# pfeiferd/genestrip

Measured on AMD Instinct MI355X. Metric: Gbp/s classified (match goal), k=31, 150bp reads; bit-exact CSV counts, higher is better.
Workload: dtype int64; 1 GPU; match: 10000000 synthetic 150 bp reads per GPU, k=31, 1911550-k-mer / 20-taxid store resident in HBM (BASELINE.json configs[1]); reads_per_gpu=10000000, read_len=150, k=31, store_kmers=1911550, store_record_bytes=67108864, store_table_bytes=131072, gate_bytes=524288, parallelism=read-sharded x1, store replicated

## Files before the change

### genestrip_amd/__init__.py

```python
from .binding import (
    GsError, lib, lib_path, device_count, abi_version, DeviceKMerStore, MatchConfig, FastqKMerMatcher,
    DeviceBloomFilter, BloomInfo, requested_mask, FastqBloomFilter, DeviceDbBuilder, DeviceDbQuality, DeviceDbUpdater, DeviceDbSizer, plan_ranges, kmer_ranges, N_COLS, N_DCOLS, N_SUMS, COLS, MEM_HOST, MEM_DEVICE,
    F_FOUND, F_RETURNED, F_COUNTED, BLOOM_XOR, BLOOM_MURMUR, BLOOM_BLOCKED, ABI_SYMBOLS, calibrate, bgzf_members, inflate_members, gunzip_device, deflate_device, deflate_reference, BGZF_EOF, DeviceDeflater, deflate_bound, DeviceReads, KrakenCounter, DeviceGenomes, DeviceView, DeviceAccessionMap, accession_slots, slot_accessions, DeviceTaxTree, read_taxids, RANK_NAMES,
    CAL_VALU_PURE, CAL_VALU_MIX, CAL_SALU, CAL_VALU_SALU, CAL_VMEM_BYTES, CAL_VMEM_WORDS, CAL_VMEM_SHARED_LINES,
    CAL_VMEM_SCATTERED, CAL_RANDOM_LINES,
)

__all__ = [
    "GsError", "lib", "lib_path", "device_count", "abi_version", "DeviceKMerStore", "MatchConfig",
    "FastqKMerMatcher", "DeviceReads", "KrakenCounter", "DeviceAccessionMap", "accession_slots", "slot_accessions", "DeviceTaxTree", "read_taxids", "RANK_NAMES", "DeviceBloomFilter", "BloomInfo", "requested_mask", "FastqBloomFilter", "DeviceDbBuilder", "DeviceDbQuality", "DeviceDbUpdater",
    "DeviceDbSizer", "DeviceGenomes", "plan_ranges", "kmer_ranges",
]
```

### genestrip_amd/binding.py

```python
import ctypes as C
import os
import sys

import numpy as np

_HERE = os.path.dirname(os.path.abspath(__file__))
_LIB = None

N_COLS, N_DCOLS, N_SUMS = 10, 4, 7
COLS = ("reads", "kmers from reads", "kmers", "unique kmers", "contigs", "contig len sq sum", "max contig length",
        "reads >=1 kmer", "reads bps", "max contig read no")
MEM_HOST, MEM_DEVICE = 0, 1
F_FOUND, F_RETURNED, F_COUNTED = 1, 2, 4
BLOOM_XOR, BLOOM_MURMUR, BLOOM_BLOCKED = 0, 1, 2

ABI_SYMBOLS = (
    "gs_last_error", "gs_strerror", "gs_device_cache_trim", "gs_abi_version", "gs_device_count",
    "gs_match_merge", "gs_match_max_contig_reads", "gs_db_create", "gs_db_get_info", "gs_db_destroy", "gs_db_save", "gs_db_load",
    "gs_match_begin", "gs_match_submit", "gs_match_submit_async", "gs_match_wait", "gs_match_sync", "gs_match_finish", "gs_match_reset", "gs_match_destroy",
    "gs_match_device_state", "gs_match_or_bitmap", "gs_match_kernel_time", "gs_match_prefilter_info", "gs_match_sn_info", "gs_match_segments",
    "gs_match_segments_fetch", "gs_match_max_counts", "gs_db_create_striped", "gs_db_create_stripe", "gs_db_stripe_export", "gs_db_stripe_attach", "gs_db_load_striped", "gs_db_load_stripe", "gs_dbbuild_begin", "gs_dbbuild_set_range", "gs_dbbuild_add", "gs_dbbuild_finish", "gs_dbbuild_fetch", "gs_dbbuild_to_db", "gs_dbbuild_destroy", "gs_db_create_part", "gs_match_encode", "gs_match_probe_keys", "gs_match_encode_route", "gs_match_route_geometry", "gs_unroute_region", "gs_match_reduce", "gs_route_keys",
    "gs_unroute_nodes",
    "gs_match_submit_text", "gs_match_submit_fasta", "gs_match_submit_fastq_ml", "gs_match_text_wait_copy", "gs_match_text_status", "gs_match_text_clear_error",
    "gs_match_text_select", "gs_match_segments_text", "gs_match_text_newlines", "gs_match_text_read_bounds", "gs_match_text_line_classes",
    "gs_pinned_alloc", "gs_pinned_free",
    "gs_filter_submit_text", "gs_filter_text_wait_copy", "gs_filter_text_status", "gs_filter_text_reset",
    "gs_filter_submit_fasta", "gs_filter_submit_fastq_ml", "gs_filter_text_read_bounds", "gs_filter_text_line_classes",
    "gs_bloom_create", "gs_bloom_build", "gs_bloom_get", "gs_bloom_destroy",
    "gs_bloom_build_db", "gs_bloom_get_info", "gs_bloom_save", "gs_bloom_load", "gs_filter_submit", "gs_filter_sync", "gs_filter_kernel_time",
    "gs_calibrate",
    "gs_match_get_device", "gs_inflate_members", "gs_inflater_create", "gs_inflater_feed", "gs_inflater_tail", "gs_gunzipper_open", "gs_gunzipper_reopen", "gs_gunzipper_next", "gs_gunzipper_info", "gs_gunzipper_first_span", "gs_gunzipper_park", "gs_gunzipper_close", "gs_gunzip_plan_device", "gs_gunzip_free", "gs_gunzip_device", "gs_text_cut_device", "gs_device_fetch", "gs_inflater_fetch", "gs_filter_get_device", "gs_inflater_reset", "gs_inflater_destroy", "gs_inflate_last_error",
    "gs_filter_compact_text", "gs_match_compact_text", "gs_filter_compact_records", "gs_match_compact_records", "gs_match_kraken_records", "gs_match_set_taxids", "gs_match_kraken_text", "gs_match_kraken_time", "gs_deflater_create", "gs_deflater_pack", "gs_deflater_info", "gs_deflater_destroy", "gs_deflater_append", "gs_deflater_pending", "gs_deflater_flush",
    "gs_deflate_bound", "gs_deflate_host", "gs_deflate_host_reference", "gs_deflate_last_error", "gs_match_text_descriptors", "gs_match_submit_fixed",
    "gs_db_value_counts", "gs_dbexport_create", "gs_dbexport_fetch", "gs_dbexport_get_device", "gs_dbexport_fastq_begin",
    "gs_dbexport_fastq_next", "gs_dbexport_destroy",
# ... 69 lines not shown
        raise GsError(-6, f"{path} is missing: build it with `make -C genestrip_amd/csrc` (hipcc, gfx950); "
                          "genestrip_amd has no CPU fallback")
    _preload_hip_runtime()
    L = C.CDLL(path)
    vp, i32, i64, dbl, ci = C.c_void_p, C.c_int32, C.c_int64, C.c_double, C.c_int
    sig = {
        "gs_last_error": (C.c_char_p, []), "gs_strerror": (C.c_char_p, [ci]), "gs_device_cache_trim": (ci, []), "gs_abi_version": (ci, []),
        "gs_device_count": (ci, [vp]),
        "gs_db_create": (ci, [vp, ci, ci, i64, vp, vp, i32, vp]), "gs_db_get_info": (ci, [vp, vp]),
        "gs_db_destroy": (ci, [vp]), "gs_db_save": (ci, [vp, C.c_char_p]), "gs_db_load": (ci, [vp, ci, C.c_char_p]),
        "gs_match_begin": (ci, [vp, vp, vp]), "gs_match_submit": (ci, [vp, vp, vp, i64, i64, ci, vp, vp]),
        "gs_match_submit_async": (ci, [vp, vp, vp, i64, i64, vp, vp, vp]), "gs_match_wait": (ci, [vp, i64]),
        "gs_match_sync": (ci, [vp]), "gs_match_finish": (ci, [vp, vp, vp]), "gs_match_reset": (ci, [vp]),
        "gs_match_destroy": (ci, [vp]), "gs_match_device_state": (ci, [vp, vp, vp, vp, vp, vp]),
        "gs_match_or_bitmap": (ci, [vp, vp, i64]), "gs_match_merge": (ci, [vp, ci]), "gs_match_max_contig_reads": (ci, [vp, vp]), "gs_match_kernel_time": (ci, [vp, vp, vp]), "gs_match_prefilter_info": (ci, [vp, vp]), "gs_match_sn_info": (ci, [vp, vp]),
        "gs_db_create_part": (ci, [vp, ci, ci, i64, vp, vp, i32, vp, ci, ci]),
        "gs_db_create_striped": (ci, [vp, vp, ci, ci, i64, vp, vp, i32, vp]),
        "gs_db_create_stripe": (ci, [vp, ci, ci, ci, ci, i64, vp, vp, i32, vp]),
        "gs_db_stripe_export": (ci, [vp, vp]),
        "gs_db_stripe_attach": (ci, [vp, ci, vp]),
        "gs_db_load_striped": (ci, [vp, vp, ci, C.c_char_p]),
        "gs_db_load_stripe": (ci, [vp, ci, ci, ci, C.c_char_p]),
        "gs_dbbuild_begin": (ci, [vp, ci, ci, i32, vp, ci, ci, ci]),
        "gs_dbbuild_add": (ci, [vp, vp, vp, vp, i64, ci, ci]),
        "gs_dbbuild_set_range": (ci, [vp, C.c_uint64, C.c_uint64]),
        "gs_dbbuild_finish": (ci, [vp, vp]),
        "gs_dbbuild_fetch": (ci, [vp, vp, vp]),
        "gs_dbbuild_to_db": (ci, [vp, vp]),
        "gs_dbbuild_destroy": (ci, [vp]),
        "gs_dbquality_begin": (ci, [vp, vp, ci, ci, ci]),
# ... 141 lines not shown
def _check(rc):
    if rc != 0:
        raise GsError(rc, (lib().gs_last_error() or b"").decode(errors="replace"))


def abi_version():
    return lib().gs_abi_version()


def device_count():
    n = C.c_int(0)
    rc = lib().gs_device_count(C.byref(n))
    return n.value if rc == 0 else 0


class InflateMember(C.Structure):
    _fields_ = [("payload_offset", C.c_int64), ("payload_len", C.c_uint32), ("isize", C.c_uint32), ("crc32", C.c_uint32),
                ("reserved", C.c_uint32)]


def bgzf_members(data):
    import struct
    b = bytes(data) if not isinstance(data, (bytes, bytearray)) else data
    out, o, n = [], 0, len(b)
    while o + 28 <= n and b[o] == 0x1f and b[o + 1] == 0x8b and b[o + 2] == 8 and (b[o + 3] & 4):
        if b[o + 3] & ~4:
            break
        xlen = struct.unpack_from("<H", b, o + 10)[0]
        q, bsize = o + 12, None
        while q + 4 <= o + 12 + xlen:
# ... 940 lines not shown
    def kernel_time(self):
        n, ms = C.c_int64(0), C.c_double(0)
        _check(lib().gs_match_kernel_time(self.h, C.byref(n), C.byref(ms)))
        return n.value, ms.value

    def prefilter_info(self):
        info = (C.c_int64 * 4)()
        _check(lib().gs_match_prefilter_info(self.h, info))
        return {"built": bool(info[0]), "n_lmers": int(info[1]), "survivors": int(info[2]), "reads": int(info[3])}

    def sn_info(self):
        info = (C.c_int64 * 3)()
        _check(lib().gs_match_sn_info(self.h, info))
        return {"deferred": bool(info[0]), "booked": int(info[1]), "rows": int(info[2])}

    def close(self):
        if getattr(self, "h", None):
            lib().gs_match_destroy(self.h)
            self.h = None

    def __del__(self):
        try:
            self.close()
        except Exception:
            pass


class BloomInfo(C.Structure):
    _fields_ = [("kind", C.c_int32), ("k", C.c_int32), ("n_hashes", C.c_int32), ("pad", C.c_int32), ("bits", C.c_int64),
                ("n_words", C.c_int64), ("expected_insertions", C.c_int64), ("n_inserted", C.c_int64), ("fpp", C.c_double)]
# ... 622 lines not shown
```

### genestrip_amd/csrc/gs_api.cpp

```cpp
#include <hip/hip_runtime.h>
#include <sys/mman.h>
#include <unistd.h>

#include <algorithm>
#include <atomic>
#include <chrono>
#include <cmath>
#include <cstdio>
#include <cstdlib>
#include <cstring>
#include <memory>
#include <string>
#include <thread>
#include <utility>
#include <vector>

#include "gs_absmod.h"
#include "gs_checksum.h"
#include "gs_indexfile.h"
#include "gs_launch.h"
#include "gs_layout.h"
#include "gs_params.h"
#include "gs_prefilter.h"
#include "gs_taxparse.h"
// ... 2052 lines not shown
    u64 *d_stat_rec_count = nullptr;
    size_t stat_recs_cap = 0;
    int32_t *d_stat_vi = nullptr;
    size_t stat_vi_cap = 0;
    bool use_stat_recs = false;
    GsQuotTable *d_quot = nullptr, *h_quot = nullptr;
    hipEvent_t quot_copied = nullptr;
    int pf_mode = -1;
    uint32_t *pf_h = nullptr;
    int64_t pf_slot_reads[4] = {0, 0, 0, 0};
    bool pf_slot_pending[4] = {false, false, false, false};
    int64_t pf_batches = 0;
    int pf_pause = 0;
    int64_t pf_last_survivors = -1, pf_last_reads = 0;
    int pf_last_slot = -1;
    int sn_mode = -1;
    bool sn_lds = false;
    GsSnRec *d_sn_recs = nullptr;
    size_t sn_recs_cap = 0;
    uint16_t *d_sn_nodes = nullptr;
    size_t sn_nodes_cap = 0;
    uint32_t *d_sn_list = nullptr;
    size_t sn_list_cap = 0;
    bool sn_last = false;
    int quot_max = 0;
    double quot_tax = 0, quot_class = 0;
    int stat_copies = 1;
    bool stats_spread = false;
    uint32_t *d_hit_counts = nullptr;
    uint32_t *d_bitmap = nullptr;
// ... 524 lines not shown
        for (int b = 0; b < 2; b++) {
            stage_free(g.bank[b]);
            if (g.copied[b]) hipEventDestroy(g.copied[b]);
        }
        for (hipEvent_t ev : g.finished)
            if (ev) hipEventDestroy(ev);
    }
    if (run->stream) hipStreamDestroy(run->stream);
    delete run;
}

#define GS_PF_MAX_PASS 0.5
#define GS_PF_HIT_RICH 0.85
#define GS_PF_PAUSE 15
#define GS_PF_SLOTS 4
static bool prefilter_rule(const gs_db *db, int mode, int samples) {
    if (mode == 0 || !db->d_pf || db->pf_set < 0) return false;
    if (mode > 0) return true;
    return 1.0 - std::pow(1.0 - (double)db->pf_set / (double)(1LL << 29), (double)samples) < GS_PF_MAX_PASS;
}
static bool prefilter_eligible(const gs_db *db) { return db->d_rec != nullptr && !db->striped() && db->n_parts <= 1 && db->info.k >= GS_MIN_K; }

static int db_ensure_prefilter(gs_db *db, int mode) {
    if (mode == 0 || db->pf_set >= 0 || !prefilter_eligible(db)) return GS_OK;
    const size_t l1_words = (size_t)1 << (GS_PF_L1_BITS - 5);
    hipStream_t stream = nullptr;
    HIP_TRY(hipStreamCreateWithFlags(&stream, hipStreamNonBlocking));
    u64 *d_count = nullptr;
    u64 count = 0;
    hipError_t e = gs_dev_alloc((void **)&db->d_pf, sizeof(uint32_t) * (GS_PF_L2_WORDS + l1_words));
    if (e == hipSuccess) e = gs_dev_alloc((void **)&d_count, sizeof(u64));
    if (e == hipSuccess) e = hipMemsetAsync(db->d_pf, 0, sizeof(uint32_t) * (GS_PF_L2_WORDS + l1_words), stream);
    if (e == hipSuccess) e = hipMemsetAsync(d_count, 0, sizeof(u64), stream);
    if (e == hipSuccess) {
// ... 33 lines not shown
    if (cfg->max_paths < 1 || cfg->max_paths > 128) return fail(GS_E_INVALID, "max_paths must be in [1,128] (C/GSConfigKey.java:350)");
    HIP_TRY(hipSetDevice(db->device));
    if (!db->complete()) return fail(GS_E_STATE, "striped store: not every stripe is attached yet (gs_db_stripe_attach)");
    if (cfg->count_unique && db->unique_owner && !db->striped())
        return fail(GS_E_STATE, "this store already has an active unique-counting run (the seen bits live in the table)");
    int pf_mode = -1;
    if (const char *ev = getenv("GS_PREFILTER")) pf_mode = atoi(ev) != 0 ? 1 : 0;
    {
        const int prc = db_ensure_prefilter(db, pf_mode);
        if (prc) return prc;
    }
    gs_run *run = new gs_run();
    run->db = db;
    run->cfg = *cfg;
    run->pf_mode = pf_mode;
    if (const char *ev = getenv("GS_SN_DEFER")) run->sn_mode = atoi(ev) != 0 ? 1 : 0;
    const size_t nv = (size_t)db->info.n_values;
    run->bitmap_words = (db->n_slots() + 31) / 32 + db->n_rec;
    hipError_t e = hipStreamCreateWithFlags(&run->stream, hipStreamNonBlocking);
    const char *force_global = getenv("GS_FORCE_GLOBAL_STATS");
    if (nv > GS_NV_LDS || (force_global != nullptr && atoi(force_global) != 0)) {
        int copies = 16;
        if (const char *ev = getenv("GS_STAT_COPIES")) copies = std::max(1, std::min(64, atoi(ev)));
        while (copies > 1 && (size_t)copies * nv * 96 > ((size_t)64 << 20)) copies /= 2;
        run->stat_copies = copies;
        run->use_stat_recs = nv <= GS_STAT_REC_MAX_VALUES;
        if (const char *ev = getenv("GS_STAT_RECS")) run->use_stat_recs = run->use_stat_recs && atoi(ev) != 0;
    }
    else {
        run->stat_copies = 16;
// ... 192 lines not shown
        if (run->db->info.n_values > 640 && (rc = grow(&run->d_stat_vi, &run->stat_vi_cap, (size_t)rec_room, run->stream))) return rc;
        if (!run->d_stat_rec_count) HIP_TRY(gs_dev_alloc((void **)&run->d_stat_rec_count, sizeof(u64)));
        HIP_TRY(hipMemsetAsync(run->d_stat_rec_count, 0, sizeof(u64), run->stream));
        P.stat_recs = run->d_stat_recs;
        P.stat_rec_count = (unsigned long long *)run->d_stat_rec_count;
    }
    const bool huge = !d_nodes && (off_stride != 0 || fixed_len - run->db->info.k + 1 >= run->huge_min);
    const bool no_queues = off_stride == 0 && !d_nodes && fixed_len - run->db->info.k + 1 <= 128 && !huge;
    if (!no_queues) HIP_TRY(hipMemsetAsync(run->d_long_count, 0, 6 * sizeof(unsigned int), run->stream));
    if (huge && (rc = ensure_huge(run, &P))) return rc;
    run->pf_last_survivors = -1;
    run->pf_last_reads = n_reads;
    run->pf_last_slot = -1;
    bool prefilter = P.quot != nullptr && fixed_len - run->db->info.k + 1 >= 65 && !d_skip && no_queues &&
                     prefilter_rule(run->db, run->pf_mode, gs_pf_samples(fixed_len, run->db->info.k));
    if (prefilter && run->pf_mode < 0) {
        for (int i = 0; i < GS_PF_SLOTS; i++)
            if (run->pf_slot_pending[i] && run->pf_h[i] != 0xffffffffu) {
                run->pf_slot_pending[i] = false;
                if ((double)run->pf_h[i] > GS_PF_HIT_RICH * (double)run->pf_slot_reads[i]) run->pf_pause = GS_PF_PAUSE;
            }
        if (run->pf_pause > 0) {
            run->pf_pause--;
            prefilter = false;
        }
    }
    run->sn_last = false;
    if (P.quot != nullptr && run->sn_lds && run->sn_mode != 0 && run->cfg.max_paths <= 64 && P.db.n_parts <= 1 && !d_skip &&
        P.db.n_values <= GS_SN_CODE_MAX && grow(&run->d_sn_recs, &run->sn_recs_cap, (size_t)n_reads, run->stream) == GS_OK &&
        grow(&run->d_sn_list, &run->sn_list_cap, (size_t)n_reads, run->stream) == GS_OK &&
        grow(&run->d_sn_nodes, &run->sn_nodes_cap, (size_t)n_reads * GS_SN_ROW, run->stream) == GS_OK) {
        P.sn_recs = run->d_sn_recs;
        P.sn_nodes = run->d_sn_nodes;
        run->sn_last = true;
    }
    int pf_slot = -1;
    if (prefilter) {
        if (!run->pf_h) {
            HIP_TRY(hipHostMalloc((void **)&run->pf_h, sizeof(uint32_t) * GS_PF_SLOTS, hipHostMallocDefault));
            for (int i = 0; i < GS_PF_SLOTS; i++) run->pf_h[i] = 0;
        }
    }
    if (prefilter || P.sn_recs)
        HIP_TRY(hipMemsetAsync(run->d_long_count + (prefilter ? 6 : 7), 0, sizeof(unsigned int) * ((prefilter ? 1 : 0) + (P.sn_recs ? 2 : 0)), run->stream));
    if ((rc = timer_start(run->timer, run->cfg.profile != 0, run->stream))) return rc;
    if (prefilter) {
        GsPrefilterParams F{};
        F.seq = d_seq;
        F.n_reads = n_reads;
// ... 2637 lines not shown
    return GS_OK;
}

extern "C" int gs_match_sn_info(gs_run *run, int64_t *info) {
    if (!run || !info) return fail(GS_E_INVALID, "NULL argument");
    HIP_TRY(hipSetDevice(run->db->device));
    HIP_TRY(hipStreamSynchronize(run->stream));
    info[0] = run->sn_last ? 1 : 0;
    info[1] = info[2] = 0;
    if (run->sn_last) {
        uint32_t n[2] = {0, 0};
        HIP_TRY(hipMemcpy(n, run->d_long_count + 7, sizeof(n), hipMemcpyDeviceToHost));
        info[1] = (int64_t)n[0];
        info[2] = (int64_t)n[1];
    }
    return GS_OK;
}

extern "C" int gs_match_kernel_time(gs_run *run, int64_t *launches, double *total_ms) {
    if (!run) return fail(GS_E_INVALID, "run is NULL");
    HIP_TRY(hipSetDevice(run->db->device));
    HIP_TRY(hipStreamSynchronize(run->stream));
    int rc = timer_collect(run->timer);
    if (rc) return rc;
    if (launches) *launches = run->timer.launches;
    if (total_ms) *total_ms = run->timer.total_ms;
    return GS_OK;
}

struct gs_bloom {
// ... 2424 lines not shown
```

### genestrip_amd/csrc/gs_kernels.hip

```cpp
#include <hip/hip_runtime.h>
#include <stdint.h>

#include <algorithm>
#include <type_traits>

#include "gs_launch.h"
#include "gs_layout.h"
#include "gs_params.h"
#include "gs_wave.h"

#define GS_LONG_CHUNK 64
#define GS_LONG_NONE 0xffffffffu

#if GS_PHASE
extern "C" int gs_debug_phase(unsigned long long *out, int reset) {
    if (out && hipMemcpyFromSymbol(out, HIP_SYMBOL(gs_phase_acc), sizeof(unsigned long long) * 16) != hipSuccess) return -1;
    if (reset) {
        unsigned long long z[16] = {0};
        if (hipMemcpyToSymbol(HIP_SYMBOL(gs_phase_acc), z, sizeof(z)) != hipSuccess) return -1;
    }
    return 0;
}
#endif

// ... 23 lines not shown

__device__ __forceinline__ bool gs_anc_or_self(int a_tin, int a_tout, int x_tin) { return a_tin <= x_tin && x_tin < a_tout; }

template <typename Tree>
__device__ __forceinline__ int gs_lca(const Tree &t, int a, int b) {
    if (a == b) return a;
    if (a < 0 || b < 0) return -1;
    const int tb = t.tin[b];
    while (a >= 0 && !gs_anc_or_self(t.tin[a], t.tout[a], tb)) a = t.parent[a];
    return a;
}

__device__ __forceinline__ int gs_sc_load(const int32_t *p) { return __hip_atomic_load(p, __ATOMIC_RELAXED, __HIP_MEMORY_SCOPE_AGENT); }
__device__ __forceinline__ void gs_sc_store(int32_t *p, int v) { __hip_atomic_store(p, v, __ATOMIC_RELAXED, __HIP_MEMORY_SCOPE_AGENT); }

template <bool LONG, bool FROM_NODES, int KC, bool WIDE, bool REC, bool STRIPED, int CTX = 2, bool FIXED = false>
__device__ __forceinline__ void gs_process_read(const GsMatchParams &P, const GsStats &st, int64_t r, u64 off, int L,
                                                int lane, int (*s_dvi)[128], int (*s_dcnt)[128], int wave_in_block,
                                                int32_t *tag, int32_t *cnt, int serial, const uint32_t (&pre)[3],
                                                uint32_t *wave_g, unsigned long long *cur, u64 live1 = 0, int64_t slot = 0) {
    static_assert(!FIXED || (!LONG && !FROM_NODES), "one iteration, probed here");
    const GsDbDev &db = P.db;
    const int k = KC ? KC : db.k;
    const int max = L - k + 1;
    const uint8_t *rd = P.seq + off;
    int out_class = -1;
    int out_flags = 0;

    if (FIXED || max > 0) {
        const int64_t read_no = P.first_read_no + r;
        const u64 key_lo = ((1ULL << 40) - 1) - ((u64)read_no & ((1ULL << 40) - 1));
        const int n_iter = LONG ? (max + 127) >> 7 : 1;
        bool found = false;
        int n_miss = 0, bad_lo = 0;
        bool bad_hi = false;
        int carry_last = GS_NODE_NONE;
// ... 46 lines not shown
                const u64 pb = P.pos_off[r] + (u64)base;
#pragma unroll
                for (int s = 0; s < 2; s++) {
                    const int p = base + 64 * s + lane;
                    int v = p < max ? P.nodes[pb + 64 * s + lane] : GS_NODE_NONE;
                    if (p < max && (v >= db.n_values || v < GS_NODE_INVALID)) v = GS_NODE_MISS;
                    node[s] = v;
                }
            } else {
                const GsMark mk = {P.count_unique, P.hit_counts, STRIPED ? P.bitmap : nullptr,
                                   STRIPED ? P.bitmap + ((db.bucket_mask + 1) * GS_SLOTS_PER_BUCKET >> 5) : nullptr};
#ifndef GS_AGG_ALL
#define GS_AGG_ALL 0
#endif
                const u64 live[2] = {~0ULL, live1};
                gs_probe_planes<KC, STRIPED, CTX, (REC || GS_AGG_ALL) && !LONG, 2, FIXED>(db, Bhi, Blo, Bbad, base, max, lane, node, wave_g, mk, FIXED ? live : nullptr);
            }

            if (!LONG) GS_STAMP(5, node[0] ^ node[1])
            const u64 hit0 = __ballot(node[0] >= 0), hit1 = __ballot(node[1] >= 0);
            found = found || ((hit0 | hit1) != 0);
            n_miss += __popcll(__ballot(node[0] == GS_NODE_MISS)) + __popcll(__ballot(node[1] == GS_NODE_MISS));

            u64 m0 = hit0, m1 = hit1;
#define GS_FIRST_NODE()                                                                                   \
    {                                                                                                     \
        const int j = m0 ? __builtin_ctzll(m0) : 64 + __builtin_ctzll(m1);                                \
        one_vi = j < 64 ? gs_readlane(node[0], j) : gs_readlane(node[1], j - 64);                         \
        const u64 e0 = __ballot(node[0] == one_vi), e1 = __ballot(node[1] == one_vi);                     \
        one_cnt = __popcll(e0) + __popcll(e1);                                                            \
        m0 &= ~e0;                                                                                        \
// ... 535 lines not shown
        s_cur[wave_in_block][0] = 0;
        s_cur[wave_in_block][1] = 64;
    }
    GS_STRIPE_TABLE((const GsMatchParams *)kp0)
#if GS_PHASE
    if (lane < 16) gs_phase_row()[lane] = 0;
    __builtin_amdgcn_fence(__ATOMIC_RELEASE, "wavefront");
    __builtin_amdgcn_wave_barrier();
    gs_stamp(-1);
#endif
    constexpr bool CAN_FIX = !FROM_NODES && !WIDE && !STRIPED;
    const int fixed_L = P.fixed_len;
    const bool fixed_batch = CAN_FIX && P.off_stride == 0 && fixed_L >= 128 && fixed_L - k + 1 <= 128 && P.quot != nullptr &&
                             (!LDS_STATS || (P.sn_recs != nullptr && P.sn_nodes != nullptr));
    const u64 fixed_live1 = gs_low_mask(fixed_L - k + 1 - 64);
    auto reads = [&](auto fixed) {
        constexpr bool FIXED = decltype(fixed)::value;
        const int64_t po_step = n_waves * P.off_stride;
        const uint64_t *po = P.off + wave_id * P.off_stride;
        uint32_t trips = 0;
        typedef const __attribute__((address_space(4))) uint32_t *GsSurvPtr;
        int64_t n_trips = n_reads;
        if (P.surv_list != nullptr) n_trips = (int64_t)*(GsSurvPtr)P.surv_count;
        if (FIXED && wave_id < n_trips) trips = (uint32_t)(n_trips - wave_id - 1) / (uint32_t)n_waves + 1u;
        const GsSurvPtr sl0 = FIXED ? (GsSurvPtr)P.surv_list : nullptr;
        for (int64_t t = wave_id; FIXED ? trips != 0 : t < n_trips; t += n_waves, po += po_step, trips--) {
            GsKernargPtr kp = kp0;
#ifndef GS_KERNARG_HOISTED
            asm volatile("" : "+s"(kp));
#endif
            const GsMatchParams &Q = *(const GsMatchParams *)kp;
            int64_t r = t;
// ... 12 lines not shown
                L = (int)(po[1] - off);
            }
            GS_STAMP(0, L)
            if (!FIXED && L - k + 1 > 128) continue;
            uint32_t pre[3];
            const uint8_t *rd = Q.seq + off;
            if (FIXED) {
                pre[0] = rd[lane];
                pre[1] = rd[64 + lane];
                const uint32_t c2 = rd[128 + lane < L ? 128 + lane : L - 1];
                pre[2] = 128 + lane < L ? c2 : GS_FILL;
            } else {
#pragma unroll
                for (int w = 0; w < 3; w++) pre[w] = 64 * w + lane < L ? rd[64 * w + lane] : GS_FILL;
            }
            gs_process_read<false, FROM_NODES, KC, WIDE, !LDS_STATS, STRIPED, CTX, FIXED>(Q, st, r, off, L, lane, s_dvi, s_dcnt, wave_in_block, nullptr, nullptr, 0,
                                                                                          pre, s_g[wave_in_block], s_cur[wave_in_block], fixed_live1, t);
        }
    };
    if constexpr (CAN_FIX) {
        if (fixed_batch)
            reads(std::true_type());
        else
            reads(std::false_type());
    } else
        reads(std::false_type());
#if GS_PHASE
    __builtin_amdgcn_fence(__ATOMIC_ACQUIRE, "wavefront");
    if (lane < 15) atomicAdd(&gs_phase_acc[lane], gs_phase_row()[lane]);
#endif
    if (!LDS_STATS && P.stat_recs != nullptr) {
        __builtin_amdgcn_fence(__ATOMIC_ACQUIRE, "wavefront");
        const u64 base = s_cur[wave_in_block][0], used = s_cur[wave_in_block][1];
        if (used < 64 && (u64)lane >= used) P.stat_recs[base + (u64)lane].vi = -1;
    }
    GS_STATS_EPILOGUE()
}

template <int NS, int KC, int CTX>
__device__ __forceinline__ void gs_process_read_wide(const GsMatchParams &P, const GsStats &st, int64_t r, u64 off, int L, int lane, uint32_t *wave_g) {
    int *s_dvi = reinterpret_cast<int *>(wave_g), *s_dcnt = reinterpret_cast<int *>(wave_g) + 64 * NS;
// ... 882 lines not shown
}

template <bool FROM_NODES, int KC, bool WIDE, bool STRIPED, int CTX>
static void gs_launch_match_t(const GsMatchParams *P, int grid, size_t lds, bool lds_stats, hipStream_t stream) {
    if (lds_stats)
        hipLaunchKernelGGL((gs_match_kernel<true, FROM_NODES, KC, WIDE, STRIPED, CTX>), dim3(grid), dim3(GS_BLOCK), lds, stream, *P);
    else
        hipLaunchKernelGGL((gs_match_kernel<false, FROM_NODES, KC, WIDE, STRIPED, CTX>), dim3(grid), dim3(GS_BLOCK), lds, stream, *P);
}

extern "C" hipError_t gs_launch_match(const GsMatchParams *P, int grid, hipStream_t stream) {
    const size_t lds = gs_stats_lds_bytes(P->db.n_values);
    const bool lds_stats = P->db.n_values <= GS_NV_LDS && !gs_force_global_stats();
    const bool ctx = P->db.mgate_ctx != 0;
    if (P->sn_nodes != nullptr && (!lds_stats || P->db.n_values > GS_SN_CODE_MAX)) return hipErrorInvalidValue;
    if (P->db.n_parts > 1) {
        if (P->nodes != nullptr) return hipErrorInvalidValue;
        if (P->max_paths > 64)
            gs_launch_match_t<false, 0, true, true, 2>(P, grid, lds, lds_stats, stream);
        else if (P->db.k == 31)
            ctx ? gs_launch_match_t<false, 31, false, true, 1>(P, grid, lds, lds_stats, stream)
                : gs_launch_match_t<false, 31, false, true, 0>(P, grid, lds, lds_stats, stream);
        else
            ctx ? gs_launch_match_t<false, 0, false, true, 1>(P, grid, lds, lds_stats, stream)
                : gs_launch_match_t<false, 0, false, true, 0>(P, grid, lds, lds_stats, stream);
        return hipGetLastError();
    }
    if (P->nodes != nullptr) {
        if (P->max_paths > 64)
            gs_launch_match_t<true, 0, true, false, 0>(P, grid, lds, lds_stats, stream);
// ... 185 lines not shown
```

### genestrip_amd/csrc/gs_params.h

```cpp
#pragma once
#include <stdint.h>

#include "../../include/gsgpu.h"
#include "gs_layout.h"
#include "gs_snrec.h"

#define GS_BLOCK 256
#ifndef GS_NV_LDS
#define GS_NV_LDS 128
#endif
#define GS_NV_TREE_LDS 2048
#define GS_STAT_REC_MAX_VALUES 10240

struct GsStatRec {
    int32_t vi;
    int32_t contigs;
    int64_t kmers;
    int64_t sq;
    uint64_t max_key;
    int32_t counted;
    int32_t read_kmers;
    int32_t read_len;
    int32_t n_pos;
    int32_t tax_err;
// ... 11 lines not shown
    int32_t classify, count_unique, max_paths, threshold;
    double max_read_tax_err, max_read_class_err;
    int64_t *sums;
    int64_t *max_keys;
    double *dsums;
    uint32_t *bitmap;
    uint32_t *hit_counts;
    int32_t *class_vi;
    uint8_t *flags;
    unsigned int *long_count;
    uint32_t *long_list;
    const int32_t *nodes;
    const unsigned long long *pos_off;
    int32_t off_stride;
    int32_t fixed_len;
    int32_t pad0;
    int32_t stat_copies;
    const uint32_t *skip;
    const GsQuotTable *quot;
    GsStatRec *stat_recs;
    unsigned long long *stat_rec_count;
    unsigned int *huge_count;
    uint32_t *huge_list;
    struct GsHugeHead *huge_head;
    struct GsHugeChunk *huge_chunks;
    uint32_t *huge_cnt;
    uint32_t *huge_first;
    uint32_t *huge_touch;
    uint32_t *huge_fold;
    int64_t long_cap;
    int32_t wide_mask;
// ... 381 lines not shown
```

### genestrip_amd/csrc/gs_wave.h

```cpp
#pragma once
#include <hip/hip_runtime.h>
#include <stdint.h>

#include "gs_layout.h"
#include "gs_params.h"

#ifndef GS_ABLATE
#define GS_ABLATE 0
#endif

#define GS_NODE_MISS (-1)
#define GS_NODE_INVALID (-2)
#define GS_NODE_NONE (-3)

__device__ __forceinline__ int gs_lane() { return (int)__lane_id(); }
__device__ __forceinline__ int gs_readlane(int v, int l) { return __builtin_amdgcn_readlane(v, l); }
__device__ __forceinline__ int gs_rfl(int v) { return __builtin_amdgcn_readfirstlane(v); }
__device__ __forceinline__ unsigned long long gs_bitset0(unsigned long long x, int bit) {
    asm("s_bitset0_b64 %0, %1" : "+s"(x) : "s"(bit));
    return x;
}
template <int LANE>
__device__ __forceinline__ int gs_writelane(int old, int v) {
    asm("v_writelane_b32 %0, %1, %2" : "+v"(old) : "s"(v), "n"(LANE));
// ... 241 lines not shown
#pragma unroll
        for (int d = 0; d < ND; d++) g[d] = (KC || d < w) ? row[d] : 0xffffffffu;
        __builtin_amdgcn_sched_group_barrier(0x100, (ND + 1) / 2, 0);
        uint32_t mn = g[0];
#pragma unroll
        for (int d = 1; d < ND; d++) mn = g[d] < mn ? g[d] : mn;
        __builtin_amdgcn_sched_group_barrier(0x002, ND, 0);
        const int idx = (int)(mn & 0xffu) + ((TWO && s >= 2) ? 128 : 0);
        cf[s] = wave_g[CAN + idx];
        p[s] = idx - (64 * s + lane);
    }
    __builtin_amdgcn_wave_barrier();
}

__device__ __forceinline__ u64 gs_low_mask(int n) { return n >= 64 ? ~0ULL : (n <= 0 ? 0ULL : ((1ULL << n) - 1ULL)); }
template <int KC, bool STRIPED, int CTX = 2, bool AGG = false, int NS = 2, bool LIT = false>
__device__ __forceinline__ void gs_probe_planes(const GsDbDev &db, const u64 (&Bhi)[NS + 1], const u64 (&Blo)[NS + 1],
                                                const u64 (&Bbad)[NS + 1], int base, int max, int lane, int (&node)[NS],
                                                uint32_t *wave_g, const GsMark &mk, const u64 *live = nullptr) {
    static_assert(NS == 2 || !AGG, "the seen-bit accumulators are laid out for two sub-rounds");
    const int k = KC ? KC : db.k;
    const uint32_t kmask = (1u << k) - 1u;
    const uint32_t vmask2 = 2u * ((1u << db.vbits) - 1u);
    const int shift_rem = (int)db.vbits + 3;
    const uint32_t bmask = (uint32_t)db.bucket_mask;
    bool any_bad = false;
#pragma unroll
    for (int w = 0; w <= NS; w++) any_bad = any_bad || Bbad[w] != 0;
    uint32_t fhi[NS], flo[NS];
    u64 act[NS];
#pragma unroll
    for (int s = 0; s < NS; s++) {
        const u64 vm = live != nullptr ? live[s] : gs_low_mask(max - base - 64 * s);
        fhi[s] = (uint32_t)gs_funnel(Bhi[s], Bhi[s + 1], lane) & kmask;
        flo[s] = (uint32_t)gs_funnel(Blo[s], Blo[s + 1], lane) & kmask;
        act[s] = vm;
        node[s] = GS_ACT(vm) ? GS_NODE_MISS : GS_NODE_NONE;
        if (any_bad) {
            const u64 wb = __ballot(((uint32_t)gs_funnel(Bbad[s], Bbad[s + 1], lane) & kmask) != 0u) & vm;
            act[s] = vm & ~wb;
            node[s] = GS_ACT(wb) ? GS_NODE_INVALID : node[s];
        }
    }
    if (db.mgate != nullptr) {
        int mp[NS];
        uint32_t cf[NS];
        GS_STAMP(2, fhi[1] ^ flo[1])
        uint32_t rhi[NS], rlo[NS];
#pragma unroll
        for (int s = 0; s < NS; s++) {
            rhi[s] = __brev(fhi[s]) >> (32 - k);
            rlo[s] = (__brev(flo[s]) >> (32 - k)) ^ kmask;
        }
        gs_wave_minimizers<KC, NS, LIT>(Bhi, Blo, fhi, flo, rhi, rlo, k, lane, wave_g, mp, cf);
        GS_STAMP(3, cf[0] ^ cf[1])
        uint32_t gh[NS], ohi[NS], olo[NS];
        int j[NS];
#pragma unroll
        for (int s = 0; s < NS; s++) gs_min_oriented_cf(cf[s], fhi[s], flo[s], rhi[s], rlo[s], k, mp[s], gh[s], ohi[s], olo[s], j[s]);
        const bool use_hint = STRIPED || CTX == 1 || (CTX == 2 && db.mgate_ctx);
        u64 two[NS];
#pragma unroll
        for (int s = 0; s < NS; s++) two[s] = ~0ULL;
        if ((GS_ABLATE & 4) == 0) {
            uint32_t gw[NS];
            uint32_t gk[NS];
#pragma unroll
            for (int s = 0; s < NS; s++) gk[s] = (CTX == 1 || (CTX == 2 && db.mgate_ctx)) ? gs_gate_ctx_key(gh[s], ohi[s], olo[s], j[s], k) : gh[s];
#pragma unroll
            for (int s = 0; s < NS; s++)
                gw[s] = db.mgate[GS_ACT(act[s]) ? ((CTX == 1 || (CTX == 2 && db.mgate_ctx)) ? gs_mgate_word_ctx(gk[s], db.mgate_bits) : gs_mgate_word(gk[s], db.mgate_bits)) : 0u];
#pragma unroll
            for (int s = 0; s < NS; s++) {
                const uint32_t bits = gs_mgate_bits(gk[s]);
                act[s] &= __ballot((gw[s] & bits) == bits);
                if (use_hint) two[s] = __ballot((gw[s] & gs_mgate_hint(gk[s])) != 0u);
            }
            GS_STAMP(4, gw[0] ^ gw[1])
        }
        if (GS_ABLATE & 6) {
#pragma unroll
            for (int s = 0; s < NS; s++)
                if (GS_ACT(act[s]) && (gh[s] ^ ohi[s] ^ olo[s] ^ (uint32_t)j[s]) == 0x12345u) node[s] = 0;
            return;
        }
        if (STRIPED || db.rec != nullptr) {
            u64 any_act = 0;
#pragma unroll
            for (int s = 0; s < NS; s++) any_act |= act[s];
            if (any_act == 0) return;
            if (AGG && mk.count_unique) {
#pragma unroll
                for (int q = 0; q < 5; q++) wave_g[64 * q + lane] = 0u;
                __builtin_amdgcn_fence(__ATOMIC_RELEASE, "wavefront");
                __builtin_amdgcn_wave_barrier();
            }
#pragma unroll
            for (int s = 0; s < NS; s++) {
                bool pending = false;
                if (GS_ACT(act[s])) {
                    const uint32_t jj = (uint32_t)j[s];
// ... 102 lines not shown
```

### include/gsgpu.h

```cpp
#ifndef GSGPU_H
#define GSGPU_H

#include <stdint.h>
#include <stddef.h>

#ifdef __cplusplus
extern "C" {
#endif

#define GS_ABI_VERSION 3

enum {
    GS_OK = 0,
    GS_E_INVALID = -1,
    GS_E_NOMEM = -2,
    GS_E_HIP = -3,
    GS_E_UNSUPPORTED = -4,
    GS_E_STATE = -5,
    GS_E_NODEVICE = -6,
    GS_E_IO = -7,
    GS_E_CANCELLED = -8
};

enum { GS_MEM_HOST = 0, GS_MEM_DEVICE = 1, GS_MEM_DEVICE_TEXT = 2  };
// ... 228 lines not shown
int gs_unroute_nodes(gs_run *run, const uint64_t *keys, const uint32_t *idx, const int32_t *back, int64_t n_routed,
                     int32_t *nodes, int64_t n_keys);

int gs_match_segments(gs_run *run, const uint8_t *seq, const uint64_t *offsets, int64_t n_reads, int mem,
                      uint64_t *seg_off);
int gs_match_segments_fetch(gs_run *run, int32_t *codes, int32_t *starts);
int gs_match_segments_text(gs_run *run, uint64_t *seg_off);
int gs_match_text_newlines(gs_run *run, uint32_t *newlines);
int gs_match_text_descriptors(gs_run *run, const int64_t *records, int32_t n, uint8_t *out, int32_t stride);
int gs_match_text_read_bounds(gs_run *run, uint64_t *bounds);

int gs_match_kernel_time(gs_run *run, int64_t *launches, double *total_ms);

int gs_match_prefilter_info(gs_run *run, int64_t *info);
int gs_match_sn_info(gs_run *run, int64_t *info);
int gs_match_get_device(gs_run *run, int *device);

typedef struct gs_bloom gs_bloom;
enum { GS_BLOOM_XOR = 0, GS_BLOOM_MURMUR = 1, GS_BLOOM_BLOCKED = 2 };

int gs_bloom_create(gs_bloom **out, int device, int kind, int64_t bits, int32_t n_hashes,
                    const int64_t *hash_factors, const uint64_t *words, int64_t n_words);
int gs_bloom_build(gs_bloom **out, int device, int kind, const int64_t *kmers, int64_t n_kmers, int mem, int64_t expected_insertions,
                   double fpp);
int gs_bloom_get(gs_bloom *bloom, int64_t *bits, int32_t *n_hashes, int64_t *hash_factors, uint64_t *words, int64_t n_words);
int gs_bloom_destroy(gs_bloom *bloom);

int gs_bloom_build_db(gs_bloom **out, gs_db *db, int kind, const uint8_t *requested,
                      int64_t expected_insertions, double fpp, int64_t *n_inserted);

// ... 189 lines not shown
```

Baseline: 375.0 Gbp/s.

## Skip the membership gate probe when the prefilter already predicts few survivors

```diff
diff --git a/genestrip_amd/__init__.py b/genestrip_amd/__init__.py
--- a/genestrip_amd/__init__.py
+++ b/genestrip_amd/__init__.py
@@ -1,5 +1,5 @@
 from .binding import (
-    GsError, lib, lib_path, device_count, abi_version, DeviceKMerStore, MatchConfig, FastqKMerMatcher,
+    GsError, lib, lib_path, device_count, gate_rule, abi_version, DeviceKMerStore, MatchConfig, FastqKMerMatcher,
     DeviceBloomFilter, BloomInfo, requested_mask, FastqBloomFilter, DeviceDbBuilder, DeviceDbQuality, DeviceDbUpdater, DeviceDbSizer, plan_ranges, kmer_ranges, N_COLS, N_DCOLS, N_SUMS, COLS, MEM_HOST, MEM_DEVICE,
     F_FOUND, F_RETURNED, F_COUNTED, BLOOM_XOR, BLOOM_MURMUR, BLOOM_BLOCKED, ABI_SYMBOLS, calibrate, bgzf_members, inflate_members, gunzip_device, deflate_device, deflate_reference, BGZF_EOF, DeviceDeflater, deflate_bound, DeviceReads, KrakenCounter, DeviceGenomes, DeviceView, DeviceAccessionMap, accession_slots, slot_accessions, DeviceTaxTree, read_taxids, RANK_NAMES,
     CAL_VALU_PURE, CAL_VALU_MIX, CAL_SALU, CAL_VALU_SALU, CAL_VMEM_BYTES, CAL_VMEM_WORDS, CAL_VMEM_SHARED_LINES,
diff --git a/genestrip_amd/binding.py b/genestrip_amd/binding.py
--- a/genestrip_amd/binding.py
+++ b/genestrip_amd/binding.py
@@ -18,7 +18,7 @@
     "gs_last_error", "gs_strerror", "gs_device_cache_trim", "gs_abi_version", "gs_device_count",
     "gs_match_merge", "gs_match_max_contig_reads", "gs_db_create", "gs_db_get_info", "gs_db_destroy", "gs_db_save", "gs_db_load",
     "gs_match_begin", "gs_match_submit", "gs_match_submit_async", "gs_match_wait", "gs_match_sync", "gs_match_finish", "gs_match_reset", "gs_match_destroy",
-    "gs_match_device_state", "gs_match_or_bitmap", "gs_match_kernel_time", "gs_match_prefilter_info", "gs_match_sn_info", "gs_match_segments",
+    "gs_match_device_state", "gs_match_or_bitmap", "gs_match_kernel_time", "gs_match_prefilter_info", "gs_match_sn_info", "gs_match_gate_info", "gs_match_gate_rule", "gs_match_segments",
     "gs_match_segments_fetch", "gs_match_max_counts", "gs_db_create_striped", "gs_db_create_stripe", "gs_db_stripe_export", "gs_db_stripe_attach", "gs_db_load_striped", "gs_db_load_stripe", "gs_dbbuild_begin", "gs_dbbuild_set_range", "gs_dbbuild_add", "gs_dbbuild_finish", "gs_dbbuild_fetch", "gs_dbbuild_to_db", "gs_dbbuild_destroy", "gs_db_create_part", "gs_match_encode", "gs_match_probe_keys", "gs_match_encode_route", "gs_match_route_geometry", "gs_unroute_region", "gs_match_reduce", "gs_route_keys",
     "gs_unroute_nodes",
     "gs_match_submit_text", "gs_match_submit_fasta", "gs_match_submit_fastq_ml", "gs_match_text_wait_copy", "gs_match_text_status", "gs_match_text_clear_error",
@@ -118,6 +118,7 @@
         "gs_match_sync": (ci, [vp]), "gs_match_finish": (ci, [vp, vp, vp]), "gs_match_reset": (ci, [vp]),
         "gs_match_destroy": (ci, [vp]), "gs_match_device_state": (ci, [vp, vp, vp, vp, vp, vp]),
         "gs_match_or_bitmap": (ci, [vp, vp, i64]), "gs_match_merge": (ci, [vp, ci]), "gs_match_max_contig_reads": (ci, [vp, vp]), "gs_match_kernel_time": (ci, [vp, vp, vp]), "gs_match_prefilter_info": (ci, [vp, vp]), "gs_match_sn_info": (ci, [vp, vp]),
+        "gs_match_gate_info": (ci, [vp, vp, vp]), "gs_match_gate_rule": (ci, [i64, ci, ci, vp]),
         "gs_db_create_part": (ci, [vp, ci, ci, i64, vp, vp, i32, vp, ci, ci]),
         "gs_db_create_striped": (ci, [vp, vp, ci, ci, i64, vp, vp, i32, vp]),
         "gs_db_create_stripe": (ci, [vp, ci, ci, ci, ci, i64, vp, vp, i32, vp]),
@@ -289,6 +290,12 @@
     return n.value if rc == 0 else 0
 
 
+def gate_rule(n_lmers, samples, mode=-1):
+    p = C.c_double(0)
+    g = lib().gs_match_gate_rule(int(n_lmers), int(samples), int(mode), C.byref(p))
+    return bool(g), p.value
+
+
 class InflateMember(C.Structure):
     _fields_ = [("payload_offset", C.c_int64), ("payload_len", C.c_uint32), ("isize", C.c_uint32), ("crc32", C.c_uint32),
                 ("reserved", C.c_uint32)]
@@ -1259,6 +1266,11 @@
         _check(lib().gs_match_sn_info(self.h, info))
         return {"deferred": bool(info[0]), "booked": int(info[1]), "rows": int(info[2])}
 
+    def gate_info(self):
+        g, p = C.c_int(0), C.c_double(0)
+        _check(lib().gs_match_gate_info(self.h, C.byref(g), C.byref(p)))
+        return {"gateless": bool(g.value), "predicted_pass": p.value}
+
     def close(self):
         if getattr(self, "h", None):
             lib().gs_match_destroy(self.h)
diff --git a/genestrip_amd/csrc/gs_api.cpp b/genestrip_amd/csrc/gs_api.cpp
--- a/genestrip_amd/csrc/gs_api.cpp
+++ b/genestrip_amd/csrc/gs_api.cpp
@@ -2090,6 +2090,9 @@
     int pf_pause = 0;
     int64_t pf_last_survivors = -1, pf_last_reads = 0;
     int pf_last_slot = -1;
+    int gate_mode = -1;
+    bool gate_last_gateless = false;
+    double gate_last_pass = -1.0;
     int sn_mode = -1;
     bool sn_lds = false;
     GsSnRec *d_sn_recs = nullptr;
@@ -2644,10 +2647,21 @@
 #define GS_PF_HIT_RICH 0.85
 #define GS_PF_PAUSE 15
 #define GS_PF_SLOTS 4
+static double prefilter_pass(int64_t n_lmers, int samples) {
+    if (n_lmers < 0) return 1.0;
+    return 1.0 - std::pow(1.0 - (double)n_lmers / (double)(1LL << 29), (double)samples);
+}
 static bool prefilter_rule(const gs_db *db, int mode, int samples) {
     if (mode == 0 || !db->d_pf || db->pf_set < 0) return false;
     if (mode > 0) return true;
-    return 1.0 - std::pow(1.0 - (double)db->pf_set / (double)(1LL << 29), (double)samples) < GS_PF_MAX_PASS;
+    return prefilter_pass(db->pf_set, samples) < GS_PF_MAX_PASS;
+}
+#define GS_PF_NOGATE_MAX_PASS 0.2
+extern "C" int gs_match_gate_rule(int64_t n_lmers, int samples, int mode, double *predicted_pass) {
+    const double pass = prefilter_pass(n_lmers, samples);
+    if (predicted_pass) *predicted_pass = pass;
+    if (mode == 0 || mode == 1) return mode == 0 ? 1 : 0;
+    return pass < GS_PF_NOGATE_MAX_PASS ? 1 : 0;
 }
 static bool prefilter_eligible(const gs_db *db) { return db->d_rec != nullptr && !db->striped() && db->n_parts <= 1 && db->info.k >= GS_MIN_K; }
 
@@ -2711,6 +2725,7 @@
     run->db = db;
     run->cfg = *cfg;
     run->pf_mode = pf_mode;
+    if (const char *ev = getenv("GS_PF_GATE")) run->gate_mode = atoi(ev) != 0 ? 1 : 0;
     if (const char *ev = getenv("GS_SN_DEFER")) run->sn_mode = atoi(ev) != 0 ? 1 : 0;
     const size_t nv = (size_t)db->info.n_values;
     run->bitmap_words = (db->n_slots() + 31) / 32 + db->n_rec;
@@ -2933,6 +2948,7 @@
     run->pf_last_slot = -1;
     bool prefilter = P.quot != nullptr && fixed_len - run->db->info.k + 1 >= 65 && !d_skip && no_queues &&
                      prefilter_rule(run->db, run->pf_mode, gs_pf_samples(fixed_len, run->db->info.k));
+    bool paused = false;
     if (prefilter && run->pf_mode < 0) {
         for (int i = 0; i < GS_PF_SLOTS; i++)
             if (run->pf_slot_pending[i] && run->pf_h[i] != 0xffffffffu) {
@@ -2942,6 +2958,7 @@
         if (run->pf_pause > 0) {
             run->pf_pause--;
             prefilter = false;
+            paused = true;
         }
     }
     run->sn_last = false;
@@ -2952,6 +2969,14 @@
         P.sn_recs = run->d_sn_recs;
         P.sn_nodes = run->d_sn_nodes;
         run->sn_last = true;
+    }
+    run->gate_last_gateless = false;
+    run->gate_last_pass = -1.0;
+    if (P.quot != nullptr && !d_nodes && !d_skip && P.db.n_parts <= 1 && run->cfg.max_paths <= 64 && !P.db.mgate_ctx &&
+        P.db.mgate != nullptr && P.db.rec != nullptr && prefilter_eligible(run->db) && (!run->sn_lds || P.sn_recs != nullptr)) {
+        const int gateless = gs_match_gate_rule(run->db->pf_set, gs_pf_samples(fixed_len, run->db->info.k), run->gate_mode, &run->gate_last_pass);
+        run->gate_last_gateless = gateless != 0 && (run->gate_mode == 0 || prefilter || paused);
+        P.fixed_nogate = run->gate_last_gateless ? 1 : 0;
     }
     int pf_slot = -1;
     if (prefilter) {
@@ -5619,6 +5644,13 @@
         info[1] = (int64_t)n[0];
         info[2] = (int64_t)n[1];
     }
+    return GS_OK;
+}
+
+extern "C" int gs_match_gate_info(gs_run *run, int *gateless, double *predicted_pass) {
+    if (!run || !gateless || !predicted_pass) return fail(GS_E_INVALID, "NULL argument");
+    *gateless = run->gate_last_gateless ? 1 : 0;
+    *predicted_pass = run->gate_last_pass;
     return GS_OK;
 }
 
diff --git a/genestrip_amd/csrc/gs_kernels.hip b/genestrip_amd/csrc/gs_kernels.hip
--- a/genestrip_amd/csrc/gs_kernels.hip
+++ b/genestrip_amd/csrc/gs_kernels.hip
@@ -61,12 +61,13 @@
 __device__ __forceinline__ int gs_sc_load(const int32_t *p) { return __hip_atomic_load(p, __ATOMIC_RELAXED, __HIP_MEMORY_SCOPE_AGENT); }
 __device__ __forceinline__ void gs_sc_store(int32_t *p, int v) { __hip_atomic_store(p, v, __ATOMIC_RELAXED, __HIP_MEMORY_SCOPE_AGENT); }
 
-template <bool LONG, bool FROM_NODES, int KC, bool WIDE, bool REC, bool STRIPED, int CTX = 2, bool FIXED = false>
+template <bool LONG, bool FROM_NODES, int KC, bool WIDE, bool REC, bool STRIPED, int CTX = 2, bool FIXED = false, bool NOGATE = false>
 __device__ __forceinline__ void gs_process_read(const GsMatchParams &P, const GsStats &st, int64_t r, u64 off, int L,
                                                 int lane, int (*s_dvi)[128], int (*s_dcnt)[128], int wave_in_block,
                                                 int32_t *tag, int32_t *cnt, int serial, const uint32_t (&pre)[3],
                                                 uint32_t *wave_g, unsigned long long *cur, u64 live1 = 0, int64_t slot = 0) {
     static_assert(!FIXED || (!LONG && !FROM_NODES), "one iteration, probed here");
+    static_assert(!NOGATE || FIXED, "the gate-less probe belongs to the FIXED loop (gs_probe_planes)");
     const GsDbDev &db = P.db;
     const int k = KC ? KC : db.k;
     const int max = L - k + 1;
@@ -143,7 +144,7 @@
 #define GS_AGG_ALL 0
 #endif
                 const u64 live[2] = {~0ULL, live1};
-                gs_probe_planes<KC, STRIPED, CTX, (REC || GS_AGG_ALL) && !LONG, 2, FIXED>(db, Bhi, Blo, Bbad, base, max, lane, node, wave_g, mk, FIXED ? live : nullptr);
+                gs_probe_planes<KC, STRIPED, CTX, (REC || GS_AGG_ALL) && !LONG, 2, FIXED, NOGATE>(db, Bhi, Blo, Bbad, base, max, lane, node, wave_g, mk, FIXED ? live : nullptr);
             }
 
             if (!LONG) GS_STAMP(5, node[0] ^ node[1])
@@ -709,8 +710,11 @@
     const bool fixed_batch = CAN_FIX && P.off_stride == 0 && fixed_L >= 128 && fixed_L - k + 1 <= 128 && P.quot != nullptr &&
                              (!LDS_STATS || (P.sn_recs != nullptr && P.sn_nodes != nullptr));
     const u64 fixed_live1 = gs_low_mask(fixed_L - k + 1 - 64);
-    auto reads = [&](auto fixed) {
+    constexpr bool CAN_NOGATE = CAN_FIX && CTX == 0;
+    const bool nogate_batch = CAN_NOGATE && fixed_batch && P.fixed_nogate != 0 && P.db.mgate != nullptr && P.db.rec != nullptr;
+    auto reads = [&](auto fixed, auto nogate) {
         constexpr bool FIXED = decltype(fixed)::value;
+        constexpr bool NOGATE = decltype(nogate)::value;
         const int64_t po_step = n_waves * P.off_stride;
         const uint64_t *po = P.off + wave_id * P.off_stride;
         uint32_t trips = 0;
@@ -753,17 +757,23 @@
 #pragma unroll
                 for (int w = 0; w < 3; w++) pre[w] = 64 * w + lane < L ? rd[64 * w + lane] : GS_FILL;
             }
-            gs_process_read<false, FROM_NODES, KC, WIDE, !LDS_STATS, STRIPED, CTX, FIXED>(Q, st, r, off, L, lane, s_dvi, s_dcnt, wave_in_block, nullptr, nullptr, 0,
+            gs_process_read<false, FROM_NODES, KC, WIDE, !LDS_STATS, STRIPED, CTX, FIXED, NOGATE>(Q, st, r, off, L, lane, s_dvi, s_dcnt, wave_in_block, nullptr, nullptr, 0,
                                                                                           pre, s_g[wave_in_block], s_cur[wave_in_block], fixed_live1, t);
         }
     };
     if constexpr (CAN_FIX) {
-        if (fixed_batch)
-            reads(std::true_type());
-        else
-            reads(std::false_type());
+        if (fixed_batch) {
+            if constexpr (CAN_NOGATE) {
+                if (nogate_batch)
+                    reads(std::true_type(), std::true_type());
+                else
+                    reads(std::true_type(), std::false_type());
+            } else
+                reads(std::true_type(), std::false_type());
+        } else
+            reads(std::false_type(), std::false_type());
     } else
-        reads(std::false_type());
+        reads(std::false_type(), std::false_type());
 #if GS_PHASE
     __builtin_amdgcn_fence(__ATOMIC_ACQUIRE, "wavefront");
     if (lane < 15) atomicAdd(&gs_phase_acc[lane], gs_phase_row()[lane]);
@@ -1676,6 +1686,11 @@
     const bool lds_stats = P->db.n_values <= GS_NV_LDS && !gs_force_global_stats();
     const bool ctx = P->db.mgate_ctx != 0;
     if (P->sn_nodes != nullptr && (!lds_stats || P->db.n_values > GS_SN_CODE_MAX)) return hipErrorInvalidValue;
+    if (P->fixed_nogate != 0 &&
+        (P->db.n_parts > 1 || P->nodes != nullptr || P->max_paths > 64 || ctx || P->db.mgate == nullptr || P->db.rec == nullptr ||
+         P->off_stride != 0 || P->quot == nullptr || P->fixed_len < 128 || P->fixed_len - P->db.k + 1 > 128 ||
+         (lds_stats && (P->sn_recs == nullptr || P->sn_nodes == nullptr))))
+        return hipErrorInvalidValue;
     if (P->db.n_parts > 1) {
         if (P->nodes != nullptr) return hipErrorInvalidValue;
         if (P->max_paths > 64)
diff --git a/genestrip_amd/csrc/gs_params.h b/genestrip_amd/csrc/gs_params.h
--- a/genestrip_amd/csrc/gs_params.h
+++ b/genestrip_amd/csrc/gs_params.h
@@ -49,7 +49,7 @@
     const unsigned long long *pos_off;
     int32_t off_stride;
     int32_t fixed_len;
-    int32_t pad0;
+    int32_t fixed_nogate;
     int32_t stat_copies;
     const uint32_t *skip;
     const GsQuotTable *quot;
diff --git a/genestrip_amd/csrc/gs_wave.h b/genestrip_amd/csrc/gs_wave.h
--- a/genestrip_amd/csrc/gs_wave.h
+++ b/genestrip_amd/csrc/gs_wave.h
@@ -279,11 +279,12 @@
 }
 
 __device__ __forceinline__ u64 gs_low_mask(int n) { return n >= 64 ? ~0ULL : (n <= 0 ? 0ULL : ((1ULL << n) - 1ULL)); }
-template <int KC, bool STRIPED, int CTX = 2, bool AGG = false, int NS = 2, bool LIT = false>
+template <int KC, bool STRIPED, int CTX = 2, bool AGG = false, int NS = 2, bool LIT = false, bool NOGATE = false>
 __device__ __forceinline__ void gs_probe_planes(const GsDbDev &db, const u64 (&Bhi)[NS + 1], const u64 (&Blo)[NS + 1],
                                                 const u64 (&Bbad)[NS + 1], int base, int max, int lane, int (&node)[NS],
                                                 uint32_t *wave_g, const GsMark &mk, const u64 *live = nullptr) {
     static_assert(NS == 2 || !AGG, "the seen-bit accumulators are laid out for two sub-rounds");
+    static_assert(!NOGATE || (LIT && !STRIPED && CTX == 0 && NS == 2), "every other variant uses the hint bits of the gate word");
     const int k = KC ? KC : db.k;
     const uint32_t kmask = (1u << k) - 1u;
     const uint32_t vmask2 = 2u * ((1u << db.vbits) - 1u);
@@ -307,7 +308,7 @@
             node[s] = GS_ACT(wb) ? GS_NODE_INVALID : node[s];
         }
     }
-    if (db.mgate != nullptr) {
+    if (NOGATE || db.mgate != nullptr) {
         int mp[NS];
         uint32_t cf[NS];
         GS_STAMP(2, fhi[1] ^ flo[1])
@@ -327,7 +328,7 @@
         u64 two[NS];
 #pragma unroll
         for (int s = 0; s < NS; s++) two[s] = ~0ULL;
-        if ((GS_ABLATE & 4) == 0) {
+        if (!NOGATE && (GS_ABLATE & 4) == 0) {
             uint32_t gw[NS];
             uint32_t gk[NS];
 #pragma unroll
@@ -349,7 +350,7 @@
                 if (GS_ACT(act[s]) && (gh[s] ^ ohi[s] ^ olo[s] ^ (uint32_t)j[s]) == 0x12345u) node[s] = 0;
             return;
         }
-        if (STRIPED || db.rec != nullptr) {
+        if (NOGATE || STRIPED || db.rec != nullptr) {
             u64 any_act = 0;
 #pragma unroll
             for (int s = 0; s < NS; s++) any_act |= act[s];
diff --git a/include/gsgpu.h b/include/gsgpu.h
--- a/include/gsgpu.h
+++ b/include/gsgpu.h
@@ -266,6 +266,8 @@
 
 int gs_match_prefilter_info(gs_run *run, int64_t *info);
 int gs_match_sn_info(gs_run *run, int64_t *info);
+int gs_match_gate_info(gs_run *run, int *gateless, double *predicted_pass);
+int gs_match_gate_rule(int64_t n_lmers, int samples, int mode, double *predicted_pass);
 int gs_match_get_device(gs_run *run, int *device);
 
 typedef struct gs_bloom gs_bloom;
```

Measured after the change: 402.0 Gbp/s, median of 6. 7.2% higher.
